# bowang-lab/BioReason

Measured on AMD Instinct MI355X. Metric: GRPO samples/sec (NT-500M+Qwen3-1.7B, DNA 2x1024, prompt 2180, gen 256), higher is better.
Workload: dtype bf16

## Files before the change

### bioreason_amd/csrc/bra_lora_plan.h

```cpp
#pragma once
#include "bra_dropout.h"

namespace bra {

inline bool lora_drop_ok(float p, long rows, long cols, int r, int nt, int R) {
    if (!(p >= 0.f && p < 1.f) || rows * cols >= (1l << 32) || nt < 1) return false;
    if (r == 32) return (R == 32 || R == 64 || R == 128) && nt <= R / 32;
    return (r == 8 || r == 16 || r == 64 || r == 128) && nt <= 3 && R == (nt * r + 63) / 64 * 64;
}

inline DropCfg make_cfg(float p, const unsigned* seeds, int n) {
    DropCfg d;
    d.thr16 = drop_threshold(p);
    d.inv_keep = 1.f / (1.f - p);
    for (int j = 0; j < 4; ++j) d.seed[j] = j < n ? seeds[j] : 0u;
    return d;
}

struct LoraSlice { int r, c0, Rs, j0, nts; };

template <class F>
inline int lora_for_slices(int r, int nt, int R, F&& f) {
    for (int c0 = 0; c0 < R; c0 += 128) {
        const int Rs = R - c0 < 128 ? R - c0 : 128;
        const int rc = f(LoraSlice{r, c0, Rs, r >= 64 ? c0 / r : 0, r >= 64 ? Rs / r : nt});
        if (rc) return rc;
    }
    return 0;
}

#define BRA_LORA_ROWS(X)                                                                                                     \
    X(s.r == 32 && s.Rs == 32, 1, 1, 32, 1)                                                                                  \
    X(s.r == 32 && s.Rs == 64 && s.nts == 1, 2, 1, 32, 1)                                                                    \
    X(s.r == 32 && s.Rs == 64 && s.nts == 2, 2, 2, 32, 2)                                                                    \
    X(s.r == 32 && s.Rs == 128 && s.nts == 3, 4, 3, 32, 3)                                                                   \
         \
    X(s.r == 32 && s.Rs == 128, 4, 4, 32, 4)                                                                                 \
    X(s.r == 8 && s.nts == 1, 2, 1, 8, 1)                                                                                    \
    X(s.r == 8 && s.nts == 2, 2, 1, 8, 2)                                                                                    \
    X(s.r == 8 && s.nts == 3, 2, 1, 8, 3)                                                                                    \
    X(s.r == 16 && s.nts == 1, 2, 1, 16, 1)                                                                                  \
    X(s.r == 16 && s.nts == 2, 2, 1, 16, 2)                                                                                  \
    X(s.r == 16 && s.nts == 3, 2, 2, 16, 3)                                                                                  \
    X(s.r == 64 && s.Rs == 64, 2, 2, 64, 1)                                                                                  \
    X(s.r == 64 && s.Rs == 128, 4, 4, 64, 2)                                                                                 \
    X(s.r == 128, 4, 4, 128, 1)

}
```

### bioreason_amd/csrc/k_lora.hip

```cpp
#include "bra_device.h"
#include "bra_api_internal.h"
#include "bra_lora_plan.h"

namespace bra {

struct LoraDownArgs {
    const bf16_t* x; long ldx;
    const bf16_t* A; long lda;
    bf16_t* t; long ldt;
    int M, K, R;
    float alpha;
    DropCfg d;
    int nb_live;
    int steps_per;
    float* part;
};

template <int RB, int NL, int TR = 32, int NT = NL>
__global__ __launch_bounds__(256) void lora_down_drop_kernel(LoraDownArgs g) {
    static_assert(TR == 8 || TR == 16 || TR == 32 || TR == 64 || TR == 128, "adapter ranks with dropout");
    static_assert(NL == (NT * TR + 31) / 32 && NL <= RB && NT <= 4, "live blocks = the blocks the targets cover");
    constexpr int KS = 128, XP = KS + 8;
    constexpr int XS_ELEMS = 2 * 32 * XP, AS_ELEMS = 2 * 32 * NL * XP;
    constexpr int RED_BYTES = 3 * NL * 64 * 16 * 4, STAGE_BYTES = (XS_ELEMS + AS_ELEMS) * 2;
    __shared__ __attribute__((aligned(16))) char lds[STAGE_BYTES > RED_BYTES ? STAGE_BYTES : RED_BYTES];
    bf16_t* xs = reinterpret_cast<bf16_t*>(lds);
    bf16_t* as = xs + XS_ELEMS;
    float* red = reinterpret_cast<float*>(lds);
    const int tid = (int)threadIdx.x, lane = tid & 63, wave = tid >> 6, h = lane >> 5;
    const int m0 = (int)blockIdx.x * 32;
    const int nstep = (g.K + KS - 1) / KS;
    const u32x4 zero4 = {0u, 0u, 0u, 0u};
    u32x4 rx[2], ra[2 * NL];
    auto issue = [&](int s) {
#pragma unroll
        for (int i = 0; i < 2; ++i) {
            const int c = tid + 256 * i, row = c >> 4, k = KS * s + 8 * (c & 15);
            int m = m0 + row; m = m < g.M ? m : g.M - 1;
            rx[i] = ld16(g.x + (long)m * g.ldx + (k < g.K ? k : 0));
        }
#pragma unroll
        for (int i = 0; i < 2 * NL; ++i) {
            const int c = tid + 256 * i, row = c >> 4, k = KS * s + 8 * (c & 15);
            ra[i] = ld16(g.A + (long)(row < g.R ? row : g.R - 1) * g.lda + (k < g.K ? k : 0));
        }
    };
    auto commit = [&](int buf, int s) {
#pragma unroll
        for (int i = 0; i < 2; ++i) {
            const int c = tid + 256 * i, k = KS * s + 8 * (c & 15);
            st16(&xs[buf * 32 * XP + (c >> 4) * XP + 8 * (c & 15)], k < g.K ? rx[i] : zero4);
        }
#pragma unroll
        for (int i = 0; i < 2 * NL; ++i) {
            const int c = tid + 256 * i, row = c >> 4, k = KS * s + 8 * (c & 15);
            st16(&as[buf * 32 * NL * XP + (c >> 4) * XP + 8 * (c & 15)], (k < g.K && row < g.R) ? ra[i] : zero4);
        }
    };
    f32x16 acc[NL];
#pragma unroll
    for (int rb = 0; rb < NL; ++rb)
#pragma unroll
        for (int q = 0; q < 16; ++q) acc[rb][q] = 0.f;
    const int s_lo = (int)blockIdx.y * g.steps_per;
    const int s_hi = s_lo + g.steps_per < nstep ? s_lo + g.steps_per : nstep;
    issue(s_lo); commit(s_lo & 1, s_lo);
    __syncthreads();
    const int mrow = m0 + (lane & 31);
    for (int s = s_lo; s < s_hi; ++s) {
        const int buf = s & 1;
        issue(s + 1 < s_hi ? s + 1 : s);
        sched_fence();
        const int lrow = opaque_i(lane & 31);
#pragma unroll
        for (int k2 = 0; k2 < 2; ++k2) {
            const int kk = 2 * wave + k2;
            const u32x4 xf = ld16(&xs[buf * 32 * XP + lrow * XP + 16 * kk + 8 * h]);
            const uint32_t e0 = (uint32_t)mrow * (uint32_t)g.K + (uint32_t)(KS * s + 16 * kk + 8 * h);
            if constexpr (TR == 32) {
#pragma unroll
                for (int rb = 0; rb < NL; ++rb) {
                    const u32x4 af = drop_apply8(xf, g.d.seed[rb], e0, g.d.thr16, g.d.inv_keep);
                    const u32x4 bf = ld16(&as[buf * 32 * NL * XP + (32 * rb + lrow) * XP + 16 * kk + 8 * h]);
                    acc[rb] = mfma_32x32x16(af, bf, acc[rb]);
                }
            } else if constexpr (TR > 32) {
#pragma unroll
                for (int jt = 0; jt < NT; ++jt) {
                    const u32x4 af = drop_apply8(xf, g.d.seed[jt], e0, g.d.thr16, g.d.inv_keep);
#pragma unroll
                    for (int b = 0; b < TR / 32; ++b) {
                        const int rb = jt * (TR / 32) + b;
                        const u32x4 bf = ld16(&as[buf * 32 * NL * XP + (32 * rb + lrow) * XP + 16 * kk + 8 * h]);
                        acc[rb] = mfma_32x32x16(af, bf, acc[rb]);
                    }
                }
            } else {
#pragma unroll
                for (int jt = 0; jt < NT; ++jt) {
                    const int rb = jt * TR / 32;
                    const u32x4 af = drop_apply8(xf, g.d.seed[jt], e0, g.d.thr16, g.d.inv_keep);
                    const u32x4 bf = ld16(&as[buf * 32 * NL * XP + (32 * rb + lrow) * XP + 16 * kk + 8 * h]);
                    acc[rb] = mfma_32x32x16(af, lrow / TR == jt % (32 / TR) ? bf : zero4, acc[rb]);
                }
            }
        }
        if (s + 1 < s_hi) commit(buf ^ 1, s + 1);
        __syncthreads();
    }
    if (wave != 0) {
#pragma unroll
        for (int rb = 0; rb < NL; ++rb)
#pragma unroll
            for (int q = 0; q < 16; ++q) red[(((wave - 1) * NL + rb) * 64 + lane) * 16 + q] = acc[rb][q];
    }
    __syncthreads();
    if (wave != 0) return;
    float* const pbase = g.part ? g.part + ((long)blockIdx.y * g.M + m0 + 4 * h) * g.R + (lane & 31) : nullptr;
    bf16_t* const tbase = g.t ? g.t + (long)(m0 + 4 * h) * g.ldt + (lane & 31) : nullptr;
#pragma unroll
    for (int rb = 0; rb < RB; ++rb) {
        const int r = 32 * rb + (lane & 31);
#pragma unroll
        for (int q = 0; q < 16; ++q) {
            const int mq = (q & 3) + 8 * (q >> 2);
            const int m = m0 + mq + 4 * h;
            float v = 0.f;
            if (rb < NL) {
                v = acc[rb < NL ? rb : 0][q];
#pragma unroll
                for (int w = 0; w < 3; ++w) v += red[((w * NL + (rb < NL ? rb : 0)) * 64 + lane) * 16 + q];
            }
            if (m < g.M && r < g.R) {
                if (g.part) pbase[(long)mq * g.R + 32 * rb] = v;
                else tbase[(long)mq * g.ldt + 32 * rb] = f2bf(g.alpha * v);
            }
        }
    }
}

__global__ __launch_bounds__(256) void lora_partial_reduce_kernel(const float* part, int ks, long MR, int R, float alpha, bf16_t* t, long ldt) {
    const long i4 = ((long)blockIdx.x * 256 + threadIdx.x) * 4;
    if (i4 >= MR) return;
    float a0 = 0.f, a1 = 0.f, a2 = 0.f, a3 = 0.f;
    for (int k = 0; k < ks; ++k) {
        const f32x4 v = *reinterpret_cast<const f32x4*>(part + (long)k * MR + i4);
        a0 += v[0]; a1 += v[1]; a2 += v[2]; a3 += v[3];
    }
    const long m = i4 / R;
    const int r = (int)(i4 - m * R);
    bf16_t* o = t + m * ldt + r;
    o[0] = f2bf(alpha * a0); o[1] = f2bf(alpha * a1); o[2] = f2bf(alpha * a2); o[3] = f2bf(alpha * a3);
}

struct LoraUpArgs {
    const bf16_t* dts; long ldd;
    const bf16_t* AT; long ldat;
    bf16_t* out; long ldo;
    int M, K, R;
    int k_chunk;
    DropCfg d;
    int nb_live;
};

template <int RB, int NL, int TR = 32, int NT = NL>
__global__ __launch_bounds__(256) void lora_up_drop_kernel(LoraUpArgs g) {
    constexpr int NC = TR == 32 ? 2 * NL : (NT * TR + 15) / 16;
    const u32x4 zero4 = {0u, 0u, 0u, 0u};
    const int lane = lane_id(), wave = (int)threadIdx.x >> 6, h = lane >> 5;
    const int m_base = ((int)blockIdx.x * 4 + wave) * 32;
    if (m_base >= g.M) return;
    int mr = m_base + (lane & 31); mr = mr < g.M ? mr : g.M - 1;
    u32x4 df[NC];
#pragma unroll
    for (int c = 0; c < NC; ++c) df[c] = ld16(g.dts + (long)mr * g.ldd + 16 * c + 8 * h);
    uint32_t rowbase[8];
    {
        const uint32_t odd0 = (uint32_t)lane & 1u;
#pragma unroll
        for (int i = 0; i < 8; ++i) {
            const int q = (int)(8 * odd0) + i;
            rowbase[i] = (uint32_t)(m_base + (q & 3) + 8 * (q >> 2) + 4 * h) * (uint32_t)g.K;
        }
    }
    const int k_lo = (int)blockIdx.y * g.k_chunk;
    int k_hi = k_lo + g.k_chunk; k_hi = k_hi < g.K ? k_hi : g.K;
    constexpr int UP_SP = 64 + 8;
    __shared__ __attribute__((aligned(16))) bf16_t stage[4][32 * UP_SP];
    bf16_t* sw = stage[wave];
    const bool vec_ok = !(g.ldo & 7) && !((size_t)g.out & 15) && !(k_lo & 7);
    for (int k0 = k_lo; k0 < k_hi; k0 += 32) {
        const int kc = k0 + (lane & 31);
        const int kr = kc < g.K ? kc : g.K - 1;
        u32x4 af[NC];
#pragma unroll
        for (int c = 0; c < NC; ++c) af[c] = ld16(g.AT + (long)kr * g.ldat + 16 * c + 8 * h);
        float o[16];
#pragma unroll
        for (int q = 0; q < 16; ++q) o[q] = 0.f;
        const uint32_t odd = (uint32_t)kr & 1u;
        const uint32_t fsh = odd ? 17u : 1u;
#pragma unroll
        for (int rb = 0; rb < NT; ++rb) {
            f32x16 acc;
#pragma unroll
            for (int q = 0; q < 16; ++q) acc[q] = 0.f;
            if constexpr (TR >= 16) {
#pragma unroll
                for (int c = rb * (TR / 16); c < (rb + 1) * (TR / 16); ++c) acc = mfma_32x32x16(df[c], af[c], acc);
            } else {
                acc = mfma_32x32x16(h == rb % 2 ? df[rb / 2] : zero4, af[rb / 2], acc);
            }
            uint32_t hh[16];
#pragma unroll
            for (int i = 0; i < 8; ++i) {
                const uint32_t mine = drop_hash(g.d.seed[rb], (rowbase[i] + (uint32_t)kr) >> 1);
                const uint32_t other = lane_swap1(mine);
                hh[i] = odd ? other : mine;
                hh[8 + i] = odd ? mine : other;
            }
#pragma unroll
            for (int q = 0; q < 16; ++q) o[q] += ((hh[q] >> fsh) & 0x7fffu) >= g.d.thr16 ? acc[q] : 0.f;
        }
        const int side = ((k0 - k_lo) >> 5) & 1;
#pragma unroll
        for (int q = 0; q < 16; ++q)
            sw[((q & 3) + 8 * (q >> 2) + 4 * h) * UP_SP + 32 * side + (lane & 31)] = kc < g.K ? f2bf(o[q] * g.d.inv_keep) : (bf16_t)0;
        if (side == 1 || k0 + 32 >= k_hi) {
            wave_lds_sync();
            const int kf = k0 - 32 * side;
            const int ncol = 32 * (side + 1);
#pragma unroll
            for (int j = 0; j < 4; ++j) {
                const int row = 8 * j + (lane >> 3), c8 = 8 * (lane & 7);
                const int m = m_base + row;
                const u32x4 v = ld16(&sw[row * UP_SP + c8]);
                if (m < g.M && c8 < ncol) {
                    bf16_t* op = g.out + (long)m * g.ldo + kf + c8;
                    if (vec_ok && kf + c8 + 8 <= g.K) st16(op, v);
                    else {
                        const bf16_t* e = reinterpret_cast<const bf16_t*>(&v);
                        for (int i = 0; i < 8; ++i) if (kf + c8 + i < g.K) op[i] = e[i];
                    }
                }
            }
            wave_lds_sync();
        }
    }
}

__global__ __launch_bounds__(256) void dropout_mask_kernel(uint8_t* out, long n, uint32_t seed, uint32_t thr16) {
    for (long i = (long)blockIdx.x * 256 + threadIdx.x; i < n; i += (long)gridDim.x * 256)
        out[i] = drop_keep1(seed, (uint32_t)i, thr16) ? 1 : 0;
}

}

using namespace bra;

extern "C" int bra_lora_down_splitk_plan(int M, int K) {
    const int gx = (M + 31) / 32, nstep = (K + 127) / 128;
    if (gx >= 192) return nstep >= 32 ? 4 : 1;
    if (gx <= 0 || nstep < 6) return 1;
    int want = 512 / gx, cap = nstep / 3;
    int ks = want < cap ? want : cap;
    if (ks < 2) return 1;
    const int per = (nstep + ks - 1) / ks;
    return (nstep + per - 1) / per;
}

extern "C" int bra_lora_down_drop(const void* x, long ldx, const void* A, long lda, void* t, long ldt, int M, int K, int R,
                                  float alpha, float p, unsigned s0, unsigned s1, unsigned s2, unsigned s3, int r, int nt,
                                  float* part, int ksplit, void* stream) {
    if (M == 0) return 0;
    if (!x || !A || !t || M < 0 || K <= 0 || K % 8 || ldx % 8 || lda % 8 || !lora_drop_ok(p, M, K, r, nt, R)) return BRA_ERR_ARG;
    if (ksplit <= 1) part = nullptr;
    else if (!part || ksplit > (K + 127) / 128 || ldt % 4) return BRA_ERR_ARG;
    const unsigned seeds[4] = {s0, s1, s2, s3};
    const int nstep = (K + 127) / 128;
    const int per = part ? (nstep + ksplit - 1) / ksplit : nstep;
    const int ny = part ? (nstep + per - 1) / per : 1;
    const dim3 grid((M + 31) / 32, ny);
    bra_stream_t st = (bra_stream_t)stream;
    return lora_for_slices(r, nt, R, [&](const LoraSlice& s) {
        float* const ps = part ? part + (long)ksplit * M * s.c0 : nullptr;
        bf16_t* const ts = (bf16_t*)t + s.c0;
        LoraDownArgs g = {(const bf16_t*)x, ldx, (const bf16_t*)A + (long)s.c0 * lda, lda, ts, ldt, M, K, s.Rs, alpha,
                          make_cfg(p, seeds + s.j0, s.nts), 0, per, ps};
#define BRA_LD(C_, RB_, NL_, TR_, NT_) if (C_) BRA_LAUNCH((lora_down_drop_kernel<RB_, NL_, TR_, NT_>), grid, dim3(256), 0, st, g); else
        BRA_LORA_ROWS(BRA_LD) return BRA_ERR_ARG;
#undef BRA_LD
        if (part) {
            const long MR = (long)M * s.Rs;
            BRA_LAUNCH(lora_partial_reduce_kernel, dim3((unsigned)((MR / 4 + 255) / 256)), dim3(256), 0, st, (const float*)ps, ny, MR, s.Rs,
                       alpha, ts, ldt);
        }
        return BRA_LAUNCH_STATUS();
    });
}

extern "C" int bra_lora_up_drop(const void* dts, long ldd, const void* AT, long ldat, void* out, long ldo, int M, int K, int R,
                                float p, unsigned s0, unsigned s1, unsigned s2, unsigned s3, int r, int nt, void* stream) {
    if (M == 0) return 0;
    if (!dts || !AT || !out || M < 0 || K <= 0 || ldd % 8 || ldat % 8 || !lora_drop_ok(p, M, K, r, nt, R)) return BRA_ERR_ARG;
    const int mblk = (M + 127) / 128;
    int splits = (1024 + mblk - 1) / mblk;
    int k_chunk = ((K + splits - 1) / splits + 31) / 32 * 32;
    k_chunk = k_chunk < 128 ? 128 : k_chunk;
    const unsigned seeds[4] = {s0, s1, s2, s3};
    LoraUpArgs g = {(const bf16_t*)dts, ldd, (const bf16_t*)AT, ldat, (bf16_t*)out, ldo, M, K, R, k_chunk, make_cfg(p, seeds, nt), 0};
    const dim3 grid(mblk, (K + k_chunk - 1) / k_chunk);
    bra_stream_t st = (bra_stream_t)stream;
#define BRA_LU(RB_, NL_, TR_, NT_) BRA_LAUNCH((lora_up_drop_kernel<RB_, NL_, TR_, NT_>), grid, dim3(256), 0, st, g)
#define BRA_LUR(TR_, NT_) BRA_LU((NT_ * TR_ + 63) / 64 * 2, (NT_ * TR_ + 31) / 32, TR_, NT_)
#define BRA_LUR3(TR_) do { if (nt == 1) BRA_LUR(TR_, 1); else if (nt == 2) BRA_LUR(TR_, 2); else BRA_LUR(TR_, 3); } while (0)
    if (r == 32 && R == 32) BRA_LU(1, 1, 32, 1);
    else if (r == 32 && R == 64) { if (nt == 1) BRA_LU(2, 1, 32, 1); else BRA_LU(2, 2, 32, 2); }
    else if (r == 32 && nt == 3) BRA_LU(4, 3, 32, 3);
    else if (r == 32) BRA_LU(4, 4, 32, 4);
    else if (r == 8) BRA_LUR3(8);
    else if (r == 16) BRA_LUR3(16);
    else if (r == 64) BRA_LUR3(64);
    else BRA_LUR3(128);
#undef BRA_LUR3
#undef BRA_LUR
#undef BRA_LU
    return BRA_LAUNCH_STATUS();
}

extern "C" int bra_dropout_mask(void* out, int M, int K, float p, unsigned seed, void* stream) {
    if (M <= 0 || K <= 0) return 0;
    if (!out || !(p >= 0.f && p < 1.f) || (long)M * K >= (1l << 32)) return BRA_ERR_ARG;
    const long n = (long)M * K;
    long grid = (n + 255) / 256; grid = grid > 4096 ? 4096 : grid;
    BRA_LAUNCH(dropout_mask_kernel, dim3((unsigned)grid), dim3(256), 0, (bra_stream_t)stream, (uint8_t*)out, n, (uint32_t)seed,
               drop_threshold(p));
    return BRA_LAUNCH_STATUS();
}
```

### bioreason_amd/csrc/k_wgrad.hip

```cpp
#include "bra_device.h"
#include "bra_api_internal.h"
#include "bra_lora_plan.h"

namespace bra {

struct WgradArgs {
    const bf16_t* Y; long ldy;
    const bf16_t* T; long ldt;
    float* C; long c_sn, c_sr;
    int M, N, R;
    int m_chunk;
    float alpha;
    DropCfg d;
    int nb_live;
};

constexpr int WG_YP = 128 + 8;

template <int RB, int DROP, int NL = RB, int RM = 0, int TR = 32, int NT = NL>
__global__ __launch_bounds__(256) void wgrad_tn_kernel(WgradArgs g) {
    static_assert(!DROP || (NL == (NT * TR + 31) / 32 && NT <= 4), "live blocks = the blocks the targets cover");
    constexpr int NYS = DROP ? NT : 2;
    __shared__ bf16_t ys[NYS][32 * WG_YP];
    constexpr int WG_TP = 32 * RB + 8, TPT = RB >= 2 ? RB / 2 : 1;
    __shared__ bf16_t ts[2][32 * WG_TP];
    const int tid = (int)threadIdx.x, lane = tid & 63, wave = tid >> 6, h = lane >> 5;
    const int n0 = (int)blockIdx.x * 128;
    const int m_lo = (int)blockIdx.y * g.m_chunk;
    int m_hi = m_lo + g.m_chunk;
    m_hi = m_hi < g.M ? m_hi : g.M;
    const int nstep = m_hi > m_lo ? (m_hi - m_lo + 31) / 32 : 0;
    const u32x4 zero4 = {0u, 0u, 0u, 0u};

    const int yr = tid >> 4, yc = (tid & 15) * 8;
    const bool ycol_ok = n0 + yc + 8 <= g.N;
    u32x4 ry[2], rt[TPT];
    auto issue = [&](int s) {
        const int m0 = m_lo + 32 * s;
#pragma unroll
        for (int i = 0; i < 2; ++i) {
            const int m = m0 + yr + 16 * i;
            const int mc = m < g.M ? m : g.M - 1;
            ry[i] = ld16(g.Y + (long)mc * g.ldy + (ycol_ok ? n0 + yc : 0));
        }
#pragma unroll
        for (int i = 0; i < TPT; ++i) {
            const int c = tid + 256 * i, tr = c / (4 * RB), tc = (c % (4 * RB)) * 8;
            const int m = m0 + (tr < 32 ? tr : 0);
            const int mc = m < g.M ? m : g.M - 1;
            rt[i] = ld16(g.T + (long)mc * g.ldt + tc);
        }
    };
    auto commit = [&](int buf, int s) {
        const int m0 = m_lo + 32 * s;
        u32x4 yv[2];
#pragma unroll
        for (int i = 0; i < 2; ++i) yv[i] = (m0 + yr + 16 * i < m_hi && ycol_ok) ? ry[i] : zero4;
        if (DROP) {
#pragma unroll
            for (int i = 0; i < 2; ++i) {
                const uint32_t e0 = (uint32_t)(m_lo + 32 * s + yr + 16 * i) * (uint32_t)g.N + (uint32_t)(n0 + yc);
#pragma unroll
                for (int jt = 0; jt < NT; ++jt)
                    st16(&ys[jt][(yr + 16 * i) * WG_YP + yc], drop_apply8(yv[i], g.d.seed[jt], e0, g.d.thr16, g.d.inv_keep));
            }
        } else {
            st16(&ys[buf][yr * WG_YP + yc], yv[0]);
            st16(&ys[buf][(yr + 16) * WG_YP + yc], yv[1]);
        }
#pragma unroll
        for (int i = 0; i < TPT; ++i) {
            const int c = tid + 256 * i, tr = c / (4 * RB), tc = (c % (4 * RB)) * 8;
            const int m = m0 + (tr < 32 ? tr : 0);
            if (tr < 32) st16(&ts[buf][tr * WG_TP + tc], m < m_hi ? rt[i] : zero4);
        }
    };

    f32x16 acc[RB];
#pragma unroll
    for (int rb = 0; rb < RB; ++rb)
#pragma unroll
        for (int r = 0; r < 16; ++r) acc[rb][r] = 0.f;

    if (nstep > 0) { issue(0); commit(0, 0); }
    __syncthreads();
    const int ncol0 = wave * 32 + (lane & 31);
    constexpr bool r_major = RM != 0;
    for (int s = 0; s < nstep; ++s) {
        const int buf = s & 1;
        issue(s + 1 < nstep ? s + 1 : s);
        sched_fence();
        const int ncol = opaque_i(ncol0);
#pragma unroll
        for (int kk = 0; kk < 2; ++kk) {
            const int mb = 16 * kk + 8 * h;
            u32x4 af0;
            if (!DROP) {
#pragma unroll
                for (int j = 0; j < 4; ++j)
                    af0[j] = (uint32_t)ys[buf][(mb + 2 * j) * WG_YP + ncol] | ((uint32_t)ys[buf][(mb + 2 * j + 1) * WG_YP + ncol] << 16);
            }
            auto y_frag = [&](int jt) {
                u32x4 f;
#pragma unroll
                for (int j = 0; j < 4; ++j)
                    f[j] = (uint32_t)ys[jt][(mb + 2 * j) * WG_YP + ncol] | ((uint32_t)ys[jt][(mb + 2 * j + 1) * WG_YP + ncol] << 16);
                return f;
            };
            auto t_frag = [&](int rb) {
                const int rc = rb * 32 + (lane & 31);
                uint32_t b[4];
#pragma unroll
                for (int j = 0; j < 4; ++j)
                    b[j] = (uint32_t)ts[buf][(mb + 2 * j) * WG_TP + rc] | ((uint32_t)ts[buf][(mb + 2 * j + 1) * WG_TP + rc] << 16);
                const u32x4 bf = {b[0], b[1], b[2], b[3]};
                return bf;
            };
            if constexpr (!DROP || TR == 32) {
#pragma unroll
                for (int rb = 0; rb < NL; ++rb) {
                    u32x4 af = af0;
                    if (DROP) af = y_frag(rb);
                    const u32x4 bf = t_frag(rb);
                    acc[rb] = r_major ? mfma_32x32x16(bf, af, acc[rb]) : mfma_32x32x16(af, bf, acc[rb]);
                }
            } else if constexpr (TR > 32) {
#pragma unroll
                for (int jt = 0; jt < NT; ++jt) {
                    const u32x4 af = y_frag(jt);
#pragma unroll
                    for (int b = 0; b < TR / 32; ++b) {
                        const int rb = jt * (TR / 32) + b;
                        const u32x4 bf = t_frag(rb);
                        acc[rb] = r_major ? mfma_32x32x16(bf, af, acc[rb]) : mfma_32x32x16(af, bf, acc[rb]);
                    }
                }
            } else {
#pragma unroll
                for (int jt = 0; jt < NT; ++jt) {
                    const int rb = jt * TR / 32;
                    const u32x4 af = y_frag(jt);
                    const u32x4 tf = t_frag(rb);
                    const u32x4 bf = (lane & 31) / TR == jt % (32 / TR) ? tf : zero4;
                    acc[rb] = r_major ? mfma_32x32x16(bf, af, acc[rb]) : mfma_32x32x16(af, bf, acc[rb]);
                }
            }
        }
        if (DROP) __syncthreads();
        if (s + 1 < nstep) commit(buf ^ 1, s + 1);
        __syncthreads();
    }
    if (nstep == 0) return;
    if (r_major) {
        const int n = n0 + wave * 32 + (lane & 31);
        float* const cb = g.C + (long)n * g.c_sn + (long)(4 * h) * g.c_sr;
#pragma unroll
        for (int rb = 0; rb < RB; ++rb)
#pragma unroll
            for (int q = 0; q < 16; ++q) {
                const int rq = rb * 32 + (q & 3) + 8 * (q >> 2);
                if (n < g.N && rq + 4 * h < g.R) atomicAdd(cb + (long)rq * g.c_sr, g.alpha * acc[rb][q]);
            }
        return;
    }
    float* const cb = g.C + (long)(n0 + wave * 32 + 4 * h) * g.c_sn + (long)(lane & 31) * g.c_sr;
#pragma unroll
    for (int rb = 0; rb < RB; ++rb) {
        const int r = rb * 32 + (lane & 31);
        if (r >= g.R) continue;
#pragma unroll
        for (int q = 0; q < 16; ++q) {
            const int nq = (q & 3) + 8 * (q >> 2);
            const int n = n0 + wave * 32 + nq + 4 * h;
            if (n < g.N) atomicAdd(cb + (long)nq * g.c_sn + (long)(32 * rb) * g.c_sr, g.alpha * acc[rb][q]);
        }
    }
}

}

using namespace bra;

static int wgrad_launch(WgradArgs& g, int m_chunk, bool drop, const LoraSlice& s, void* stream) {
    if (m_chunk <= 0) {
        const int ntile = (g.N + 127) / 128;
        int splits = (512 + ntile - 1) / ntile;
        m_chunk = (g.M + splits - 1) / splits;
        m_chunk = m_chunk < 256 ? 256 : m_chunk;
    }
    g.m_chunk = (m_chunk + 31) / 32 * 32;
    const dim3 grid((g.N + 127) / 128, (g.M + g.m_chunk - 1) / g.m_chunk);
    bra_stream_t st = (bra_stream_t)stream;
    const bool rm = g.c_sn == 1;
#define BRA_WG(C_, RB_, NL_, TR_, NT_)                                                                             \
    if (C_) {                                                                                                      \
        if (drop && rm) BRA_LAUNCH((wgrad_tn_kernel<RB_, 1, NL_, 1, TR_, NT_>), grid, dim3(256), 0, st, g);        \
        else if (drop) BRA_LAUNCH((wgrad_tn_kernel<RB_, 1, NL_, 0, TR_, NT_>), grid, dim3(256), 0, st, g);         \
        else if (rm) BRA_LAUNCH((wgrad_tn_kernel<RB_, 0, RB_, 1>), grid, dim3(256), 0, st, g);                     \
        else BRA_LAUNCH((wgrad_tn_kernel<RB_, 0, RB_, 0>), grid, dim3(256), 0, st, g);                             \
    } else
    BRA_LORA_ROWS(BRA_WG) return BRA_ERR_ARG;
#undef BRA_WG
    return BRA_LAUNCH_STATUS();
}

static int wgrad_slices(const void* Y, long ldy, const void* T, long ldt, float* C, long c_sn, long c_sr, int M, int N, int R, float alpha,
                        int m_chunk, bool drop, float p, const unsigned* seeds, int r, int nt, void* stream) {
    return lora_for_slices(r, nt, R, [&](LoraSlice s) {
        if (!drop) { s.r = 32; s.nts = s.Rs / 32; }
        WgradArgs g = {(const bf16_t*)Y, ldy, (const bf16_t*)T + s.c0, ldt, C + (long)s.c0 * c_sr, c_sn, c_sr, M, N, s.Rs, 0, alpha,
                       drop ? make_cfg(p, seeds + s.j0, s.nts) : DropCfg{}, 0};
        return wgrad_launch(g, m_chunk, drop, s, stream);
    });
}

extern "C" int bra_wgrad_tn(const void* Y, long ldy, const void* T, long ldt, float* C, long c_sn, long c_sr, int M, int N,
                            int R, float alpha, int m_chunk, void* stream) {
    if (M == 0 || N == 0) return 0;
    if (!Y || !T || !C || M < 0 || N < 0 || N % 8 || ldy % 8 || ldt % 8 || R <= 0 || (R != 32 && R % 64)) return BRA_ERR_ARG;
    return wgrad_slices(Y, ldy, T, ldt, C, c_sn, c_sr, M, N, R, alpha, m_chunk, false, 0.f, nullptr, 0, 0, stream);
}

extern "C" int bra_wgrad_tn_drop(const void* Y, long ldy, const void* T, long ldt, float* C, long c_sn, long c_sr, int M,
                                 int N, int R, float alpha, int m_chunk, float p, unsigned s0, unsigned s1, unsigned s2,
                                 unsigned s3, int r, int nt, void* stream) {
    if (M == 0 || N == 0) return 0;
    if (!Y || !T || !C || M < 0 || N < 0 || N % 8 || ldy % 8 || ldt % 8 || !lora_drop_ok(p, M, N, r, nt, R)) return BRA_ERR_ARG;
    const unsigned seeds[4] = {s0, s1, s2, s3};
    return wgrad_slices(Y, ldy, T, ldt, C, c_sn, c_sr, M, N, R, alpha, m_chunk, true, p, seeds, r, nt, stream);
}
```

### include/bioreason_hip_debug.h

```cpp
#ifndef BIOREASON_HIP_DEBUG_H
#define BIOREASON_HIP_DEBUG_H
#include "bioreason_hip.h"
#ifdef __cplusplus
extern "C" {
#endif

int bra_gemm_set_variant(int v);
int bra_gemm_set_ring_fill(int pct);
int bra_gemm_set_row_split(int on);
int bra_gemm_set_epi_lds(int on);
int bra_sample_set_one_launch(int on);
int bra_gemm_set_glds_rows(int rows);
int bra_attn_set_block_order(int legacy);
int bra_attn_set_fwd4(int on);
int bra_attn_set_bwd4(int mask);
int bra_attn_set_probe(void* buf);


int bra_dec_gemm2_probe(const void* x, long ldx, const float* ss_in, int nss_in, const void* norm_w, float eps, const void* W,
                        long ldw, const void* res, long ldres, void* out, long ldo, float* ss_out, int nss_out, int M, int N,
                        int K, int act, int out_f32, int packed, void* probe, void* stream);
int bra_debug_set_probe(void* p);

int bra_gridsync_bytes(void);
int bra_persist_layer_desc_size(void);
int bra_persist_set_stamps(void* p);
int bra_qwen_layers_persist(const void* layers_dev, int L, int R, int copies, int H, int Hq, int Hkv, int hd, int F, int P,
                            long vt_pitch, int C, long cp, float eps, float scale, const float* cosT, const float* sinT,
                            const int* pos, const float* rope_rows, const void* pmask, int t, const int* t_dev, void* x,
                            void* qkv, void* o, void* h, void* act, float* ss_ws, int nss, float* part_o, float* part_ml,
                            int nslot, void* sync, int prefetch, int stop_after, int timeout_us, void* stream);
int bra_qwen_decode_step_persist(const void* layers_host, const void* layers_dev, int L, int R, int copies, int H, int Hq, int Hkv,
                                 int hd, int F, int P, long vt_pitch, int C, long cp, int V, float eps, float scale, const void* E,
                                 const void* norm_w, const float* cosT, const float* sinT, const int* tok, const int* pos,
                                 const void* pmask, int t, const int* t_dev, int embed_done, void* x, void* qkv, void* o, void* h,
                                 void* act, float* ss_ws, int nss, float* part_o, float* part_ml, int nslot, float* logits,
                                 void* sync, int prefetch, int stop_after, int timeout_us, void* stream);
int bra_chain_probe(void* done, void* buf, void* errs, const void* wts, long wts_bytes, int nwg, int n, int chained, int wchunks,
                    int timeout_us, void* stream_a, void* stream_b);
int bra_gridbar_probe(void* sync, void* buf, void* errs, const void* wts, long wts_bytes, int nwg, int iters, int mode,
                      int wchunks, int timeout_us, void* stream);

#ifdef __cplusplus
}
#endif
#endif
```

Before: 19.68.

## Issue several K-steps of global loads ahead in LoRA down and wgrad kernels

Adds a depth parameter D to the LoRA down-projection and wgrad kernels so that D stages of global loads are kept in flight in register slots, not one step ahead. The intent is to hide global memory latency in small grids where there are too few workgroups to cover it. By default the wgrad path uses depth 8 only for dropout, row-major, rank-32 multi-target launches with small grids, while the LoRA down deep path is reachable only under a debug flag. The cost is higher register pressure from the extra staging registers.

```diff
diff --git a/bioreason_amd/csrc/bra_lora_plan.h b/bioreason_amd/csrc/bra_lora_plan.h
--- a/bioreason_amd/csrc/bra_lora_plan.h
+++ b/bioreason_amd/csrc/bra_lora_plan.h
@@ -30,20 +30,20 @@
 }
 
 #define BRA_LORA_ROWS(X)                                                                                                     \
-    X(s.r == 32 && s.Rs == 32, 1, 1, 32, 1)                                                                                  \
-    X(s.r == 32 && s.Rs == 64 && s.nts == 1, 2, 1, 32, 1)                                                                    \
-    X(s.r == 32 && s.Rs == 64 && s.nts == 2, 2, 2, 32, 2)                                                                    \
-    X(s.r == 32 && s.Rs == 128 && s.nts == 3, 4, 3, 32, 3)                                                                   \
+    X(s.r == 32 && s.Rs == 32, 1, 1, 32, 1, 8)                                                                               \
+    X(s.r == 32 && s.Rs == 64 && s.nts == 1, 2, 1, 32, 1, 8)                                                                 \
+    X(s.r == 32 && s.Rs == 64 && s.nts == 2, 2, 2, 32, 2, 4)                                                                 \
+    X(s.r == 32 && s.Rs == 128 && s.nts == 3, 4, 3, 32, 3, 4)                                                                \
          \
-    X(s.r == 32 && s.Rs == 128, 4, 4, 32, 4)                                                                                 \
-    X(s.r == 8 && s.nts == 1, 2, 1, 8, 1)                                                                                    \
-    X(s.r == 8 && s.nts == 2, 2, 1, 8, 2)                                                                                    \
-    X(s.r == 8 && s.nts == 3, 2, 1, 8, 3)                                                                                    \
-    X(s.r == 16 && s.nts == 1, 2, 1, 16, 1)                                                                                  \
-    X(s.r == 16 && s.nts == 2, 2, 1, 16, 2)                                                                                  \
-    X(s.r == 16 && s.nts == 3, 2, 2, 16, 3)                                                                                  \
-    X(s.r == 64 && s.Rs == 64, 2, 2, 64, 1)                                                                                  \
-    X(s.r == 64 && s.Rs == 128, 4, 4, 64, 2)                                                                                 \
-    X(s.r == 128, 4, 4, 128, 1)
+    X(s.r == 32 && s.Rs == 128, 4, 4, 32, 4, 3)                                                                              \
+    X(s.r == 8 && s.nts == 1, 2, 1, 8, 1, 8)                                                                                 \
+    X(s.r == 8 && s.nts == 2, 2, 1, 8, 2, 8)                                                                                 \
+    X(s.r == 8 && s.nts == 3, 2, 1, 8, 3, 8)                                                                                 \
+    X(s.r == 16 && s.nts == 1, 2, 1, 16, 1, 8)                                                                               \
+    X(s.r == 16 && s.nts == 2, 2, 1, 16, 2, 8)                                                                               \
+    X(s.r == 16 && s.nts == 3, 2, 2, 16, 3, 4)                                                                               \
+    X(s.r == 64 && s.Rs == 64, 2, 2, 64, 1, 4)                                                                               \
+    X(s.r == 64 && s.Rs == 128, 4, 4, 64, 2, 3)                                                                              \
+    X(s.r == 128, 4, 4, 128, 1, 3)
 
 }
diff --git a/bioreason_amd/csrc/k_lora.hip b/bioreason_amd/csrc/k_lora.hip
--- a/bioreason_amd/csrc/k_lora.hip
+++ b/bioreason_amd/csrc/k_lora.hip
@@ -1,6 +1,7 @@
 #include "bra_device.h"
 #include "bra_api_internal.h"
 #include "bra_lora_plan.h"
+#include <atomic>
 
 namespace bra {
 
@@ -16,11 +17,12 @@
     float* part;
 };
 
-template <int RB, int NL, int TR = 32, int NT = NL>
+template <int RB, int NL, int TR = 32, int NT = NL, int D = 0>
 __global__ __launch_bounds__(256) void lora_down_drop_kernel(LoraDownArgs g) {
     static_assert(TR == 8 || TR == 16 || TR == 32 || TR == 64 || TR == 128, "adapter ranks with dropout");
     static_assert(NL == (NT * TR + 31) / 32 && NL <= RB && NT <= 4, "live blocks = the blocks the targets cover");
-    constexpr int KS = 128, XP = KS + 8;
+    static_assert(D >= 0 && D * (2 + 2 * NL) < 64, "the requests in flight are counted by a 6-bit counter");
+    constexpr int KS = 128, XP = KS + 8, DS = D ? D : 1;
     constexpr int XS_ELEMS = 2 * 32 * XP, AS_ELEMS = 2 * 32 * NL * XP;
     constexpr int RED_BYTES = 3 * NL * 64 * 16 * 4, STAGE_BYTES = (XS_ELEMS + AS_ELEMS) * 2;
     __shared__ __attribute__((aligned(16))) char lds[STAGE_BYTES > RED_BYTES ? STAGE_BYTES : RED_BYTES];
@@ -31,30 +33,30 @@
     const int m0 = (int)blockIdx.x * 32;
     const int nstep = (g.K + KS - 1) / KS;
     const u32x4 zero4 = {0u, 0u, 0u, 0u};
-    u32x4 rx[2], ra[2 * NL];
-    auto issue = [&](int s) {
+    u32x4 rx[DS][2], ra[DS][2 * NL];
+    auto issue = [&](int slot, int s) {
 #pragma unroll
         for (int i = 0; i < 2; ++i) {
             const int c = tid + 256 * i, row = c >> 4, k = KS * s + 8 * (c & 15);
             int m = m0 + row; m = m < g.M ? m : g.M - 1;
-            rx[i] = ld16(g.x + (long)m * g.ldx + (k < g.K ? k : 0));
+            rx[slot][i] = ld16(g.x + (long)m * g.ldx + (k < g.K ? k : 0));
         }
 #pragma unroll
         for (int i = 0; i < 2 * NL; ++i) {
             const int c = tid + 256 * i, row = c >> 4, k = KS * s + 8 * (c & 15);
-            ra[i] = ld16(g.A + (long)(row < g.R ? row : g.R - 1) * g.lda + (k < g.K ? k : 0));
+            ra[slot][i] = ld16(g.A + (long)(row < g.R ? row : g.R - 1) * g.lda + (k < g.K ? k : 0));
         }
     };
-    auto commit = [&](int buf, int s) {
+    auto commit = [&](int buf, int slot, int s) {
 #pragma unroll
         for (int i = 0; i < 2; ++i) {
             const int c = tid + 256 * i, k = KS * s + 8 * (c & 15);
-            st16(&xs[buf * 32 * XP + (c >> 4) * XP + 8 * (c & 15)], k < g.K ? rx[i] : zero4);
+            st16(&xs[buf * 32 * XP + (c >> 4) * XP + 8 * (c & 15)], k < g.K ? rx[slot][i] : zero4);
         }
 #pragma unroll
         for (int i = 0; i < 2 * NL; ++i) {
             const int c = tid + 256 * i, row = c >> 4, k = KS * s + 8 * (c & 15);
-            st16(&as[buf * 32 * NL * XP + (c >> 4) * XP + 8 * (c & 15)], (k < g.K && row < g.R) ? ra[i] : zero4);
+            st16(&as[buf * 32 * NL * XP + (c >> 4) * XP + 8 * (c & 15)], (k < g.K && row < g.R) ? ra[slot][i] : zero4);
         }
     };
     f32x16 acc[NL];
@@ -64,12 +66,8 @@
         for (int q = 0; q < 16; ++q) acc[rb][q] = 0.f;
     const int s_lo = (int)blockIdx.y * g.steps_per;
     const int s_hi = s_lo + g.steps_per < nstep ? s_lo + g.steps_per : nstep;
-    issue(s_lo); commit(s_lo & 1, s_lo);
-    __syncthreads();
     const int mrow = m0 + (lane & 31);
-    for (int s = s_lo; s < s_hi; ++s) {
-        const int buf = s & 1;
-        issue(s + 1 < s_hi ? s + 1 : s);
+    auto multiply = [&](int buf, int s) {
         sched_fence();
         const int lrow = opaque_i(lane & 31);
 #pragma unroll
@@ -105,8 +103,43 @@
                 }
             }
         }
-        if (s + 1 < s_hi) commit(buf ^ 1, s + 1);
+    };
+    if constexpr (D == 0) {
+        issue(0, s_lo); commit(s_lo & 1, 0, s_lo);
         __syncthreads();
+        for (int s = s_lo; s < s_hi; ++s) {
+            const int buf = s & 1;
+            issue(0, s + 1 < s_hi ? s + 1 : s);
+            multiply(buf, s);
+            if (s + 1 < s_hi) commit(buf ^ 1, 0, s + 1);
+            __syncthreads();
+        }
+    } else {
+        const int s_last = s_hi - 1;
+#pragma unroll
+        for (int d = 0; d < D; ++d) issue(d, s_lo + d < s_last ? s_lo + d : s_last);
+        commit(s_lo & 1, 0, s_lo);
+        __syncthreads();
+        int s = s_lo;
+        for (; s + D < s_hi; s += D) {
+#pragma unroll
+            for (int d = 0; d < D; ++d) {
+                const int buf = (s + d) & 1;
+                issue(d, s + d + D < s_last ? s + d + D : s_last);
+                multiply(buf, s + d);
+                commit(buf ^ 1, (d + 1) % D, s + d + 1);
+                __syncthreads();
+            }
+        }
+#pragma unroll
+        for (int d = 0; d < D; ++d) {
+            if (s + d < s_hi) {
+                const int buf = (s + d) & 1;
+                multiply(buf, s + d);
+                if (s + d + 1 < s_hi) commit(buf ^ 1, (d + 1) % D, s + d + 1);
+                __syncthreads();
+            }
+        }
     }
     if (wave != 0) {
 #pragma unroll
@@ -257,6 +290,11 @@
 }
 
 using namespace bra;
+
+#ifdef BRA_DEBUG
+static std::atomic<int> g_lora_entry_issue{0};
+extern "C" int bra_lora_set_entry_issue(int on) { g_lora_entry_issue = on ? 1 : 0; return 0; }
+#endif
 
 extern "C" int bra_lora_down_splitk_plan(int M, int K) {
     const int gx = (M + 31) / 32, nstep = (K + 127) / 128;
@@ -287,7 +325,15 @@
         bf16_t* const ts = (bf16_t*)t + s.c0;
         LoraDownArgs g = {(const bf16_t*)x, ldx, (const bf16_t*)A + (long)s.c0 * lda, lda, ts, ldt, M, K, s.Rs, alpha,
                           make_cfg(p, seeds + s.j0, s.nts), 0, per, ps};
-#define BRA_LD(C_, RB_, NL_, TR_, NT_) if (C_) BRA_LAUNCH((lora_down_drop_kernel<RB_, NL_, TR_, NT_>), grid, dim3(256), 0, st, g); else
+#ifdef BRA_DEBUG
+#define BRA_LD(C_, RB_, NL_, TR_, NT_, D_)                                                                                  \
+        if (C_) {                                                                                                           \
+            if (g_lora_entry_issue) BRA_LAUNCH((lora_down_drop_kernel<RB_, NL_, TR_, NT_, D_>), grid, dim3(256), 0, st, g); \
+            else BRA_LAUNCH((lora_down_drop_kernel<RB_, NL_, TR_, NT_, 0>), grid, dim3(256), 0, st, g);                     \
+        } else
+#else
+#define BRA_LD(C_, RB_, NL_, TR_, NT_, D_) if (C_) BRA_LAUNCH((lora_down_drop_kernel<RB_, NL_, TR_, NT_, 0>), grid, dim3(256), 0, st, g); else
+#endif
         BRA_LORA_ROWS(BRA_LD) return BRA_ERR_ARG;
 #undef BRA_LD
         if (part) {
diff --git a/bioreason_amd/csrc/k_wgrad.hip b/bioreason_amd/csrc/k_wgrad.hip
--- a/bioreason_amd/csrc/k_wgrad.hip
+++ b/bioreason_amd/csrc/k_wgrad.hip
@@ -1,6 +1,7 @@
 #include "bra_device.h"
 #include "bra_api_internal.h"
 #include "bra_lora_plan.h"
+#include <atomic>
 
 namespace bra {
 
@@ -17,9 +18,10 @@
 
 constexpr int WG_YP = 128 + 8;
 
-template <int RB, int DROP, int NL = RB, int RM = 0, int TR = 32, int NT = NL>
+template <int RB, int DROP, int NL = RB, int RM = 0, int TR = 32, int NT = NL, int D = 0>
 __global__ __launch_bounds__(256) void wgrad_tn_kernel(WgradArgs g) {
     static_assert(!DROP || (NL == (NT * TR + 31) / 32 && NT <= 4), "live blocks = the blocks the targets cover");
+    constexpr int DS = D ? D : 1;
     constexpr int NYS = DROP ? NT : 2;
     __shared__ bf16_t ys[NYS][32 * WG_YP];
     constexpr int WG_TP = 32 * RB + 8, TPT = RB >= 2 ? RB / 2 : 1;
@@ -34,28 +36,28 @@
 
     const int yr = tid >> 4, yc = (tid & 15) * 8;
     const bool ycol_ok = n0 + yc + 8 <= g.N;
-    u32x4 ry[2], rt[TPT];
-    auto issue = [&](int s) {
+    u32x4 ry[DS][2], rt[DS][TPT];
+    auto issue = [&](int slot, int s) {
         const int m0 = m_lo + 32 * s;
 #pragma unroll
         for (int i = 0; i < 2; ++i) {
             const int m = m0 + yr + 16 * i;
             const int mc = m < g.M ? m : g.M - 1;
-            ry[i] = ld16(g.Y + (long)mc * g.ldy + (ycol_ok ? n0 + yc : 0));
+            ry[slot][i] = ld16(g.Y + (long)mc * g.ldy + (ycol_ok ? n0 + yc : 0));
         }
 #pragma unroll
         for (int i = 0; i < TPT; ++i) {
             const int c = tid + 256 * i, tr = c / (4 * RB), tc = (c % (4 * RB)) * 8;
             const int m = m0 + (tr < 32 ? tr : 0);
             const int mc = m < g.M ? m : g.M - 1;
-            rt[i] = ld16(g.T + (long)mc * g.ldt + tc);
+            rt[slot][i] = ld16(g.T + (long)mc * g.ldt + tc);
         }
     };
-    auto commit = [&](int buf, int s) {
+    auto commit = [&](int buf, int slot, int s) {
         const int m0 = m_lo + 32 * s;
         u32x4 yv[2];
 #pragma unroll
-        for (int i = 0; i < 2; ++i) yv[i] = (m0 + yr + 16 * i < m_hi && ycol_ok) ? ry[i] : zero4;
+        for (int i = 0; i < 2; ++i) yv[i] = (m0 + yr + 16 * i < m_hi && ycol_ok) ? ry[slot][i] : zero4;
         if (DROP) {
 #pragma unroll
             for (int i = 0; i < 2; ++i) {
@@ -72,7 +74,7 @@
         for (int i = 0; i < TPT; ++i) {
             const int c = tid + 256 * i, tr = c / (4 * RB), tc = (c % (4 * RB)) * 8;
             const int m = m0 + (tr < 32 ? tr : 0);
-            if (tr < 32) st16(&ts[buf][tr * WG_TP + tc], m < m_hi ? rt[i] : zero4);
+            if (tr < 32) st16(&ts[buf][tr * WG_TP + tc], m < m_hi ? rt[slot][i] : zero4);
         }
     };
 
@@ -82,13 +84,9 @@
 #pragma unroll
         for (int r = 0; r < 16; ++r) acc[rb][r] = 0.f;
 
-    if (nstep > 0) { issue(0); commit(0, 0); }
-    __syncthreads();
     const int ncol0 = wave * 32 + (lane & 31);
     constexpr bool r_major = RM != 0;
-    for (int s = 0; s < nstep; ++s) {
-        const int buf = s & 1;
-        issue(s + 1 < nstep ? s + 1 : s);
+    auto multiply = [&](int buf) {
         sched_fence();
         const int ncol = opaque_i(ncol0);
 #pragma unroll
@@ -146,9 +144,47 @@
                 }
             }
         }
-        if (DROP) __syncthreads();
-        if (s + 1 < nstep) commit(buf ^ 1, s + 1);
+    };
+    if constexpr (D == 0) {
+        if (nstep > 0) { issue(0, 0); commit(0, 0, 0); }
         __syncthreads();
+        for (int s = 0; s < nstep; ++s) {
+            const int buf = s & 1;
+            issue(0, s + 1 < nstep ? s + 1 : s);
+            multiply(buf);
+            if (DROP) __syncthreads();
+            if (s + 1 < nstep) commit(buf ^ 1, 0, s + 1);
+            __syncthreads();
+        }
+    } else {
+        if (nstep == 0) return;
+        const int s_last = nstep - 1;
+#pragma unroll
+        for (int d = 0; d < D; ++d) issue(d, d < s_last ? d : s_last);
+        commit(0, 0, 0);
+        __syncthreads();
+        int s = 0;
+        for (; s + D < nstep; s += D) {
+#pragma unroll
+            for (int d = 0; d < D; ++d) {
+                const int buf = (s + d) & 1;
+                issue(d, s + d + D < s_last ? s + d + D : s_last);
+                multiply(buf);
+                if (DROP) __syncthreads();
+                commit(buf ^ 1, (d + 1) % D, s + d + 1);
+                __syncthreads();
+            }
+        }
+#pragma unroll
+        for (int d = 0; d < D; ++d) {
+            if (s + d < nstep) {
+                const int buf = (s + d) & 1;
+                multiply(buf);
+                if (DROP) __syncthreads();
+                if (s + d + 1 < nstep) commit(buf ^ 1, (d + 1) % D, s + d + 1);
+                __syncthreads();
+            }
+        }
     }
     if (nstep == 0) return;
     if (r_major) {
@@ -180,6 +216,13 @@
 }
 
 using namespace bra;
+
+constexpr int kWgradDepth = 8;
+constexpr int wgrad_depth(int tr, int nt) { return tr == 32 && nt >= 2 ? kWgradDepth : 0; }
+#ifdef BRA_DEBUG
+static std::atomic<int> g_wgrad_entry_issue{-1};
+extern "C" int bra_wgrad_set_entry_issue(int mode) { g_wgrad_entry_issue = mode < 0 ? -1 : mode ? 1 : 0; return 0; }
+#endif
 
 static int wgrad_launch(WgradArgs& g, int m_chunk, bool drop, const LoraSlice& s, void* stream) {
     if (m_chunk <= 0) {
@@ -192,15 +235,37 @@
     const dim3 grid((g.N + 127) / 128, (g.M + g.m_chunk - 1) / g.m_chunk);
     bra_stream_t st = (bra_stream_t)stream;
     const bool rm = g.c_sn == 1;
-#define BRA_WG(C_, RB_, NL_, TR_, NT_)                                                                             \
+#ifdef BRA_DEBUG
+    const int mode = g_wgrad_entry_issue;
+#else
+    constexpr int mode = -1;
+#endif
+    const bool entry = mode != 0 && drop && rm && grid.x * grid.y <= 256;
+#define BRA_WG_DROP(RB_, NL_, TR_, NT_, WD_)                                                                       \
+        if (rm) BRA_LAUNCH((wgrad_tn_kernel<RB_, 1, NL_, 1, TR_, NT_, WD_>), grid, dim3(256), 0, st, g);           \
+        else BRA_LAUNCH((wgrad_tn_kernel<RB_, 1, NL_, 0, TR_, NT_, WD_>), grid, dim3(256), 0, st, g);
+#define BRA_WG_PLAIN(RB_, WD_)                                                                                     \
+        if (rm) BRA_LAUNCH((wgrad_tn_kernel<RB_, 0, RB_, 1, 32, RB_, WD_>), grid, dim3(256), 0, st, g);            \
+        else BRA_LAUNCH((wgrad_tn_kernel<RB_, 0, RB_, 0, 32, RB_, WD_>), grid, dim3(256), 0, st, g);
+#ifdef BRA_DEBUG
+#define BRA_WG_FORCED(RB_, NL_, TR_, NT_)                                                                          \
+        if (mode == 1) { if (drop) { BRA_WG_DROP(RB_, NL_, TR_, NT_, kWgradDepth) } else { BRA_WG_PLAIN(RB_, kWgradDepth) } } else
+#else
+#define BRA_WG_FORCED(RB_, NL_, TR_, NT_)
+#endif
+#define BRA_WG(C_, RB_, NL_, TR_, NT_, D_)                                                                         \
     if (C_) {                                                                                                      \
-        if (drop && rm) BRA_LAUNCH((wgrad_tn_kernel<RB_, 1, NL_, 1, TR_, NT_>), grid, dim3(256), 0, st, g);        \
-        else if (drop) BRA_LAUNCH((wgrad_tn_kernel<RB_, 1, NL_, 0, TR_, NT_>), grid, dim3(256), 0, st, g);         \
-        else if (rm) BRA_LAUNCH((wgrad_tn_kernel<RB_, 0, RB_, 1>), grid, dim3(256), 0, st, g);                     \
-        else BRA_LAUNCH((wgrad_tn_kernel<RB_, 0, RB_, 0>), grid, dim3(256), 0, st, g);                             \
+        BRA_WG_FORCED(RB_, NL_, TR_, NT_)                                                                          \
+        if (entry && wgrad_depth(TR_, NT_))                                                                        \
+            BRA_LAUNCH((wgrad_tn_kernel<RB_, 1, NL_, 1, TR_, NT_, wgrad_depth(TR_, NT_)>), grid, dim3(256), 0, st, g); \
+        else if (drop) { BRA_WG_DROP(RB_, NL_, TR_, NT_, 0) }                                                      \
+        else { BRA_WG_PLAIN(RB_, 0) }                                                                              \
     } else
     BRA_LORA_ROWS(BRA_WG) return BRA_ERR_ARG;
 #undef BRA_WG
+#undef BRA_WG_FORCED
+#undef BRA_WG_PLAIN
+#undef BRA_WG_DROP
     return BRA_LAUNCH_STATUS();
 }
 
diff --git a/include/bioreason_hip_debug.h b/include/bioreason_hip_debug.h
--- a/include/bioreason_hip_debug.h
+++ b/include/bioreason_hip_debug.h
@@ -15,6 +15,8 @@
 int bra_attn_set_fwd4(int on);
 int bra_attn_set_bwd4(int mask);
 int bra_attn_set_probe(void* buf);
+int bra_lora_set_entry_issue(int on);
+int bra_wgrad_set_entry_issue(int mode);
 
 
 int bra_dec_gemm2_probe(const void* x, long ldx, const float* ss_in, int nss_in, const void* norm_w, float eps, const void* W,
```

New measurement: 19.67. Within noise of the previous version (-0.0%).
